# thangktran/HardwareAwareOptimalQuantumCircuitCuttingAndKnitting

Measured on AMD Instinct MI355X. Metric: subcircuit-instances/s (full-knit wall time = ms_per_step), syc 32 p=2, higher is better.
Workload: dtype f64

## Files before the change

hardwareawareoptimalquantumcircuitcuttingandknitting_amd/_lib.py:

```python
from __future__ import annotations

import ctypes
import os
import threading

_HERE = os.path.dirname(os.path.abspath(__file__))
LIB_PATH = os.environ.get("QKNIT_LIB") or os.path.join(_HERE, "libqknit.so")

c_i32, c_i64, c_u32, c_u64 = ctypes.c_int32, ctypes.c_int64, ctypes.c_uint32, ctypes.c_uint64
c_vp, c_dp, c_lp = ctypes.c_void_p, ctypes.POINTER(ctypes.c_double), ctypes.POINTER(ctypes.c_int64)


class QkPass(ctypes.Structure):
    _fields_ = [("tile_mask", c_u64), ("group_begin", c_i32), ("group_end", c_i32),
                ("flags", c_i32), ("traced_local", c_u32)]


class QkProgram(ctypes.Structure):
    _fields_ = [("n", c_i32), ("n_eff", c_i32), ("m", c_i32), ("n_slots", c_i32),
                ("packed", c_i32), ("n_passes", c_i32), ("passes", ctypes.POINTER(QkPass)),
                ("ops", c_vp), ("groups", c_vp), ("mats", c_vp)]


class QkLowrankPlan(ctypes.Structure):
# ... 42 lines not shown
    "qk_gemm_keyed": (c_i32, [c_vp, c_i64, c_i64, c_i64, c_vp, c_i64, c_vp, c_i64, c_vp, c_i64,
                              c_vp, c_i64, c_vp, ctypes.c_int]),
    "qk_gemm_keyed_pred": (c_i32, [c_vp, c_i64, c_i64, c_i64, c_vp, c_i64, c_vp, c_i64, c_vp, c_i64,
                                   c_vp, c_i64, c_vp, ctypes.c_int, c_vp]),
    "qk_gemm_outer_paired": (c_i32, [c_vp, c_i64, c_i64, c_i64, c_vp, c_i64, c_vp, c_i64, c_vp, c_i64,
                                     c_vp, c_vp]),
    "qk_knit_outer_stream": (c_i32, [c_vp, ctypes.c_int, c_i64, c_vp, c_i64, c_vp, c_i64, ctypes.c_uint64,
                                     ctypes.c_uint64, c_vp]),
    "qk_knit_outer_stream_kind": (c_i32, [ctypes.c_int, c_i64, c_u64, c_u64, c_i64, c_i64,
                                          ctypes.POINTER(ctypes.c_int), ctypes.POINTER(ctypes.c_int)]),
    "qk_knit_outer_stream_range": (c_i32, [c_vp, ctypes.c_int, c_i64, c_vp, c_i64, c_vp, c_i64, ctypes.c_uint64,
                                           ctypes.c_uint64, c_i64, c_i64, c_vp, c_vp]),
    "qk_rank_factors": (c_i32, [c_vp, c_i64, c_vp, c_vp, ctypes.c_double, ctypes.c_double, ctypes.c_double,
                                ctypes.c_int, c_vp, c_vp, c_vp]),
    "qk_prep_workspace_bytes": (c_i32, [c_vp, c_i64, c_i64, ctypes.POINTER(c_i64)]),
    "qk_prep_operands": (c_i32, [c_vp, ctypes.c_int, ctypes.c_int, c_vp, c_vp, c_i64, c_i64, c_vp, ctypes.c_int,
                                 c_vp, c_vp, c_i64, c_i64, c_vp, c_vp, c_vp, c_vp, c_vp, c_vp, c_i64]),
    "qk_compress_operands": (c_i32, [c_vp, ctypes.c_int, ctypes.c_int, c_vp, c_vp, c_i64, c_vp, c_vp, c_vp, c_i64,
                                     c_vp]),
    "qk_compress_operands_ld": (c_i32, [c_vp, ctypes.c_int, ctypes.c_int, c_vp, c_vp, c_i64, c_i64, c_vp, c_i64, c_vp,
                                        c_vp, c_i64, c_i64, c_vp, c_i64]),
    "qk_compress_probe_v": (c_i32, [c_vp, ctypes.c_int, ctypes.c_int, c_vp, c_vp, c_i64, c_i64, c_vp, c_i64, c_vp, c_vp,
                                    c_i64, c_i64, c_vp, c_i64, c_vp, c_i64, c_vp, c_i64]),
    "qk_probe_errors_vpart": (c_i32, [c_vp, ctypes.c_int, ctypes.c_int, c_vp, c_i64, c_i64, c_vp, c_i64, c_vp, c_vp,
                                      c_i64, c_vp, c_vp, ctypes.c_double, ctypes.c_double, c_vp, c_vp, c_vp, c_i64,
                                      c_vp]),
    "qk_probe_workspace_bytes": (c_i32, [c_vp, c_i64, ctypes.POINTER(c_i64)]),
    "qk_probe_errors": (c_i32, [c_vp, ctypes.c_int, ctypes.c_int, c_vp, c_i64, c_i64, c_vp, c_i64, c_vp, c_vp, c_i64,
                                c_i64, c_vp, c_i64, c_vp, c_vp, ctypes.c_double, ctypes.c_double, c_vp, c_vp, c_vp,
                                c_i64]),
    "qk_probe_errors_tally": (c_i32, [c_vp, ctypes.c_int, ctypes.c_int, c_vp, c_i64, c_i64, c_vp, c_i64, c_vp, c_vp, c_i64,
                                c_i64, c_vp, c_i64, c_vp, c_vp, ctypes.c_double, ctypes.c_double, c_vp, c_vp, c_vp,
                                c_i64, c_vp]),
    "qk_probe_accept": (c_i32, [c_vp, c_vp, ctypes.c_int, c_vp, ctypes.c_double, ctypes.c_double, c_vp, c_vp]),
    "qk_rank_tally": (c_i32, [c_vp, c_vp, c_vp, c_vp]),
    "qk_knit_workspace_bytes": (c_i32, [ctypes.POINTER(QkKnitPlan), ctypes.POINTER(c_i64)]),
    "qk_knit": (c_i32, [c_vp, ctypes.POINTER(QkKnitPlan), c_vp, c_vp, c_i64, c_vp]),
    "qk_khatri_rao": (c_i32, [c_vp, c_i64, c_i64, c_i64, c_vp, c_i64, c_vp, c_i64, c_vp]),
    "qk_gather_rows": (c_i32, [c_vp, c_i64, c_i64, c_vp, c_vp, c_vp, c_vp]),
    "qk_npd_workspace_bytes": (c_i32, [c_i64, c_i64, ctypes.POINTER(c_i64)]),
    "qk_threshold_count": (c_i32, [c_vp, c_i64, c_vp, ctypes.c_double, c_vp, c_i64, c_vp]),
    "qk_npd": (c_i32, [c_vp, c_i64, c_vp, ctypes.c_double, c_i64, c_vp, c_i64, c_vp, c_vp, c_vp]),
    "qk_qd_from_rows": (c_i32, [c_vp, c_i64, c_i64, c_vp, c_vp, ctypes.c_double, c_vp]),
    "qk_qd_merge": (c_i32, [c_vp, c_i64, c_vp, c_vp, c_i64, c_vp, c_vp, ctypes.c_double, c_i64, c_vp]),
    "qk_qd_axpby": (c_i32, [c_vp, c_i64, ctypes.c_double, c_vp, ctypes.c_double, c_vp, ctypes.c_double, c_vp]),
    "qk_hellinger": (c_i32, [c_vp, c_i64, c_vp, c_vp, c_vp]),
# ... 64 lines not shown
```

hardwareawareoptimalquantumcircuitcuttingandknitting_amd/csrc/qknit_plan.hip:

```cpp
#include <hip/hip_runtime.h>

#include <algorithm>
#include <cstdlib>
#include <string>
#include <vector>

#include "internal.h"

namespace {

int pfail(qk_ctx* ctx, int code, const std::string& msg) {
    if (ctx) ctx->err = msg;
    return code;
}

__global__ void qk_pdep_keys_kernel(int64_t n, uint64_t mask, int64_t* keys) {
    for (int64_t x = blockIdx.x * (int64_t)blockDim.x + threadIdx.x; x < n; x += (int64_t)gridDim.x * blockDim.x) {
        uint64_t m = mask, k = 0, bit = 1;
        for (; m; m &= m - 1, bit <<= 1)
            if ((uint64_t)x & bit) k |= m & (~m + 1);
        keys[x] = (int64_t)k;
    }
}

// ... 173 lines not shown
};

int lowrank_layout(qk_ctx* ctx, const qk_lowrank_plan* p, LowrankLayout& L, std::string& why) {
    if (!p || p->terms < 2 || p->terms > 64 || (p->terms & 1) || p->rows_a < 1 || p->rows_b < 1 || !p->wt_a ||
        !p->wt_b || !p->probes || p->nbits < 2 || p->nbits > 32) {
        why = "qk_knit_lowrank: need even 2 <= terms <= 64, swept rows, transforms, probes, 2 <= nbits <= 32";
        return QK_EARG;
    }
    if (p->rows_a > INT32_MAX || p->rows_b > INT32_MAX) {
        why = "qk_knit_lowrank: rows_a and rows_b must be at most INT32_MAX";
        return QK_EARG;
    }
    const uint64_t full = (uint64_t(1) << p->nbits) - 1;
    if ((p->mask_a & p->mask_b) || (p->mask_a | p->mask_b) != full || !(p->mask_b & 1)) {
        why = "qk_knit_lowrank: masks must be disjoint, cover all nbits output bits, bit 0 in mask_b";
        return QK_EARG;
    }
    const int64_t NA = int64_t(1) << __builtin_popcountll(p->mask_a), NB = int64_t(1) << __builtin_popcountll(p->mask_b);
    if (NA % 128 || NB % 128) {
        why = "qk_knit_lowrank: each fragment needs >= 7 measured clbits (operand widths multiples of 128)";
        return QK_EARG;
    }
    const int64_t K = p->terms;
    int64_t prep = 0, probe = 0;
    int rc = qk_prep_workspace_bytes(ctx, NA, NB, &prep);
    if (!rc) rc = qk_probe_workspace_bytes(ctx, NA, &probe);
    if (rc) {
        why = "qk_knit_lowrank: workspace queries failed";
        return rc;
    }
    int64_t off = 0;
    auto take = [&](int64_t bytes) { const int64_t o = off; off += align16(bytes); return o; };
    L.xa = take(K * NA * 8);
    L.xb = take(K * NB * 8);
    L.g = take(2 * K * K * 8);
    L.u = take(K * LR_PROBES * 8);
    L.prep = take(prep);
    L.ta = take(LR_RMAX * K * 8);
    L.tb = take(LR_RMAX * K * 8);
    L.r = take(8);
    L.a2 = take(LR_RMAX * NA * 8);
    L.b2 = take(LR_RMAX * NB * 8);
    L.e2 = take(2 * LR_PROBES * 8);
    L.k = take(8);
    L.err = take(8);
    L.probe = take(probe);
    L.ka = contiguous_bits(p->mask_a) ? -1 : take(NA * 8);
    L.kb = contiguous_bits(p->mask_b) ? -1 : take(NB * 8);
    L.total = off;
// ... 18 lines not shown
    return QK_OK;
}

int qk_knit_lowrank(qk_ctx* ctx, const qk_lowrank_plan* p, const double* q_a, const double* q_b, void* workspace,
                    int64_t workspace_bytes, double* out, int32_t* rank_out) {
    if (!ctx) return QK_EARG;
    LowrankLayout L;
    std::string why;
    int rc = lowrank_layout(ctx, p, L, why);
    if (rc) return pfail(ctx, rc, why);
    if (!q_a || !q_b || !out || !workspace || workspace_bytes < L.total)
        return pfail(ctx, QK_EARG, "qk_knit_lowrank: null rows / output, or workspace below qk_knit_lowrank_workspace_bytes");
    if (hipSetDevice(ctx->device) != hipSuccess) return pfail(ctx, QK_EHIP, "qk_knit_lowrank: hipSetDevice");
    char* ws = static_cast<char*>(workspace);
    auto D = [&](int64_t off) { return reinterpret_cast<double*>(ws + off); };
    const int K = p->terms;
    const int64_t NA = int64_t(1) << __builtin_popcountll(p->mask_a), NB = int64_t(1) << __builtin_popcountll(p->mask_b);
    double *XA = D(L.xa), *XB = D(L.xb), *G = D(L.g), *U = D(L.u);
    int32_t* r = reinterpret_cast<int32_t*>(ws + L.r);
    int32_t* k = reinterpret_cast<int32_t*>(ws + L.k);
    rc = qk_prep_operands(ctx, K, (int)p->rows_a, p->wt_a, q_a, NA, NA, XA, (int)p->rows_b, p->wt_b, q_b, NB, NB, XB,
                          p->probes, G, G + K * K, U, D(L.prep), L.prep_bytes);
    if (!rc) rc = qk_rank_factors(ctx, K, G, G + K * K, p->lam_tol, p->s_tol, p->s_abs, LR_RMAX, D(L.ta), D(L.tb), r);
    if (!rc) rc = qk_compress_operands(ctx, K, LR_RMAX, D(L.ta), XA, NA, D(L.a2), D(L.tb), XB, NB, D(L.b2));
    if (!rc)
        rc = qk_probe_errors(ctx, K, LR_RMAX, XA, NA, NA, D(L.a2), NA, U, D(L.b2), NB, NB, p->probes, NB, D(L.e2), r,
                             p->rank_tol, p->rank_tol_rel, k, D(L.err), D(L.probe), L.probe_bytes);
    if (!rc)
        rc = qk_knit_outer_stream_range(ctx, p->nbits, LR_RMAX, D(L.a2), NA, D(L.b2), NB, p->mask_a, p->mask_b, 0,
                                        int64_t(1) << p->nbits, k, out);
    if (rc) return rc;
    int64_t* ka = L.ka >= 0 ? reinterpret_cast<int64_t*>(ws + L.ka) : nullptr;
    int64_t* kb = L.kb >= 0 ? reinterpret_cast<int64_t*>(ws + L.kb) : nullptr;
    if (ka) hipLaunchKernelGGL(qk_pdep_keys_kernel, dim3(grid_of(NA)), dim3(256), 0, ctx->stream, NA, p->mask_a, ka);
    if (kb) hipLaunchKernelGGL(qk_pdep_keys_kernel, dim3(grid_of(NB)), dim3(256), 0, ctx->stream, NB, p->mask_b, kb);
    const int64_t sa = ka ? 0 : int64_t(1) << __builtin_ctzll(p->mask_a);
    const int64_t sb = kb ? 0 : int64_t(1) << __builtin_ctzll(p->mask_b);
    rc = qk_gemm_keyed_pred(ctx, NA, NB, K, XA, NA, XB, NB, ka, sa, kb, sb, out, 0, k);
    if (rc) return rc;
    if (rank_out) hipLaunchKernelGGL(qk_copy_i32_kernel, dim3(1), dim3(1), 0, ctx->stream, k, rank_out);
    if (hipGetLastError() != hipSuccess) return pfail(ctx, QK_EHIP, "qk_knit_lowrank: launch failed");
    return QK_OK;
}

}
```

hardwareawareoptimalquantumcircuitcuttingandknitting_amd/csrc/qknit_prep.hip:

```cpp
#include <hip/hip_runtime.h>

#include <cstdint>
#include <string>

#include "internal.h"

namespace {

typedef double d4_t __attribute__((ext_vector_type(4)));
typedef double d2_t __attribute__((ext_vector_type(2)));

constexpr int PK = 64;
constexpr int PCT = 128;
constexpr int PNP = 16;
constexpr int PTH = 512;
constexpr int XLD = PCT + 2;
constexpr int PG_BLK = 10;
constexpr int PPG = PG_BLK * 256;
constexpr int PPA = PPG;
constexpr int PPB = PPG + PK * PNP;
__host__ __device__ constexpr int prep_tri(int bi, int bj) { return bi * 4 - bi * (bi - 1) / 2 + (bj - bi); }

struct PrepSide {
    const double* Wt;
// ... 480 lines not shown
        const double* pr = P + (int64_t)i16 * ldp;
#pragma unroll
        for (int s0 = 0; s0 < 32; s0 += VB) {
            double pb[VB];
#pragma unroll
            for (int s = 0; s < VB; ++s) {
                const int64_t col = base + 4 * (s0 + s) + k4;
                pb[s] = col < N ? pr[col] : 0.0;
            }
#pragma unroll
            for (int s = 0; s < VB; ++s) {
                const double a = i16 < 8 ? Bt[wave][i16][4 * (s0 + s) + k4] : 0.0;
                va = __builtin_amdgcn_mfma_f64_16x16x4f64(a, pb[s], va, 0, 0, 0);
            }
        }
    }
#pragma unroll
    for (int r = 0; r < 2; ++r) Vw[wave][(k4 + 4 * r) * 16 + i16] = va[r];
    __syncthreads();
    if (tid < PV_PART)
        vpart[wg * PV_PART + tid] = (Vw[0][tid] + Vw[1][tid]) + (Vw[2][tid] + Vw[3][tid]);
}

__global__ __launch_bounds__(256) void qk_probe_v_kernel(int rmax, const double* __restrict__ B2, int64_t ldb2,
                                                         int64_t NB, const double* __restrict__ P, int64_t ldp,
                                                         double* __restrict__ vpart) {
    const int tid = threadIdx.x, lane = tid & 63, wave = tid >> 6;
    double acc[8][4];
#pragma unroll
    for (int jj = 0; jj < 8; ++jj)
#pragma unroll
        for (int q = 0; q < 4; ++q) acc[jj][q] = 0.0;
    struct Col {
        double b[8], pv[4];
    };
    const int64_t step = (int64_t)gridDim.x * 64;
    auto fetch = [&](int64_t c, Col& x) {
        const int64_t cc = c < NB ? c : NB - 1;
#pragma unroll
        for (int jj = 0; jj < 8; ++jj) x.b[jj] = B2[(int64_t)min(jj, rmax - 1) * ldb2 + cc];
#pragma unroll
        for (int q = 0; q < 4; ++q) x.pv[q] = P[(int64_t)(4 * wave + q) * ldp + cc];
    };
    auto mac = [&](const Col& x) {
#pragma unroll
        for (int jj = 0; jj < 8; ++jj)
// ... 91 lines not shown
            acc = __builtin_amdgcn_mfma_f64_16x16x4f64(a2[jj], Vs[4 * jj + l4][l16], acc, 0, 0, 0);
#pragma unroll
        for (int rr = 0; rr < 4; ++rr) e2 = fma(acc[rr], acc[rr], e2);
    }
    e2 += __shfl_xor(e2, 16, 64);
    e2 += __shfl_xor(e2, 32, 64);
    f2 += __shfl_xor(f2, 16, 64);
    f2 += __shfl_xor(f2, 32, 64);
    if (l4 == 0) {
        ep[wave][l16] = e2;
        ep[wave][PNP + l16] = f2;
    }
    __syncthreads();
    if (tid < 2 * PNP)
        epart[(int64_t)blockIdx.x * 2 * PNP + tid] = ep[0][tid] + ep[1][tid] + ep[2][tid] + ep[3][tid];
}

constexpr int PE = 2 * PNP;

__global__ __launch_bounds__(256) void qk_probe_accept_kernel(const double* __restrict__ epart, int n,
                                                              const int32_t* __restrict__ r_dev, double tol,
                                                              double rel_tol, double* __restrict__ e2_out,
                                                              int32_t* __restrict__ k_out, double* __restrict__ err_out,
                                                              int64_t* __restrict__ tally = nullptr) {
    __shared__ double acc[256];
    const int tid = threadIdx.x, p = tid % PE;
    constexpr int STEP = 256 / PE;
    double s8[8] = {0, 0, 0, 0, 0, 0, 0, 0};
    int b = tid / PE;
    for (; b + 31 * STEP < n; b += 32 * STEP) {
        double v[32];
#pragma unroll
        for (int u = 0; u < 32; ++u) v[u] = epart[(int64_t)(b + u * STEP) * PE + p];
#pragma unroll
        for (int u = 0; u < 32; ++u) s8[u & 7] += v[u];
    }
    for (; b < n; b += STEP) s8[0] += epart[(int64_t)b * PE + p];
    const double s = ((s8[0] + s8[1]) + (s8[2] + s8[3])) + ((s8[4] + s8[5]) + (s8[6] + s8[7]));
    acc[tid] = s;
    __syncthreads();
    for (int w = 128; w >= PE; w >>= 1) {
        if (tid < w) acc[tid] += acc[tid + w];
        __syncthreads();
    }
    if (tid < PE && e2_out) e2_out[tid] = acc[tid];
    if (tid == 0 && k_out) {
        double m = 0.0, f = 0.0;
        for (int q = 0; q < PNP; ++q) {
            m = fmax(m, acc[q]);
            f = fmax(f, acc[PNP + q]);
        }
        const double err = sqrt(m);
        const double bound = fmax(tol, rel_tol * sqrt(f));
        const int r = *r_dev;
        if (err_out) *err_out = err;
        const int k = (r > 0 && err <= bound) ? r : 0;
        *k_out = k;
        if (tally) {
            tally[0] += r == 0 ? 1 : 0;
// ... 114 lines not shown
                        double* B2, int64_t ldb2, const double* probes, int64_t ldp, double* vpart,
                        int64_t vpart_doubles) {
    if (!ctx) return QK_EARG;
    if (K < 1 || K > PK || rmax < 1 || rmax > 8 || NA < 2 || NB < 2 || (NA | NB | ldxa | lda2 | ldxb | ldb2) & 1)
        return fail(ctx, QK_EARG, "qk_compress_probe_v: need 1 <= K <= 64, 1 <= rmax <= 8, even widths and strides");
    if (ldxa < NA || lda2 < NA || ldxb < NB || ldb2 < NB || ldp < NB)
        return fail(ctx, QK_EARG, "qk_compress_probe_v: leading dimension below the width");
    if (!TA || !XA || !A2 || !TB || !XB || !B2 || !probes || !vpart)
        return fail(ctx, QK_EARG, "qk_compress_probe_v: null buffer");
    if ((reinterpret_cast<uintptr_t>(XA) | reinterpret_cast<uintptr_t>(XB) | reinterpret_cast<uintptr_t>(A2) |
         reinterpret_cast<uintptr_t>(B2)) & 15)
        return fail(ctx, QK_EARG, "qk_compress_probe_v: operands must be 16-B aligned");
    const int64_t ga = (NA + CV_COLS - 1) / CV_COLS, gb = (NB + CV_COLS - 1) / CV_COLS;
    if (vpart_doubles < gb * PV_PART) return fail(ctx, QK_EARG, "qk_compress_probe_v: vpart too small");
    if (hipSetDevice(ctx->device) != hipSuccess) return fail(ctx, QK_EHIP, "qk_compress_probe_v: hipSetDevice");
    hipLaunchKernelGGL(qk_compress_v_kernel, dim3((unsigned)(ga + gb)), dim3(256), 0, ctx->stream, K, rmax, TA, XA, NA,
                       ldxa, A2, lda2, TB, XB, NB, ldxb, B2, ldb2, probes, ldp, vpart, (int)ga);
    const hipError_t e = hipGetLastError();
    if (e != hipSuccess)
        return fail(ctx, QK_EHIP, (std::string("qk_compress_probe_v: ") + hipGetErrorString(e)).c_str());
    return QK_OK;
}

int qk_probe_errors_vpart(qk_ctx* ctx, int K, int rmax, const double* XA, int64_t ldx, int64_t NA, const double* A2,
                          int64_t lda2, const double* U, const double* vpart, int64_t gv, double* e2,
                          const int32_t* r_dev, double tol, double rel_tol, int32_t* k_out, double* err_out,
                          double* work, int64_t work_bytes, int64_t* tally) {
    if (!ctx) return QK_EARG;
    if (K < 1 || K > PK || rmax < 1 || rmax > 8 || NA < 16 || NA % 16 || gv < 1)
        return fail(ctx, QK_EARG, "qk_probe_errors_vpart: need 1 <= K <= 64, 1 <= rmax <= 8, NA % 16 == 0, gv >= 1");
    if (!XA || !A2 || !U || !vpart || !work || (k_out && !r_dev) || (tally && !k_out))
        return fail(ctx, QK_EARG, "qk_probe_errors_vpart: null buffer");
    if (ldx < NA) return fail(ctx, QK_EARG, "qk_probe_errors_vpart: leading dimension");
    const int gd = probe_grid_d(ctx, NA);
    if (work_bytes < (int64_t)(PV_GRID * PV_PART + gd * PE) * (int64_t)sizeof(double))
        return fail(ctx, QK_EARG, "qk_probe_errors_vpart: workspace too small (qk_probe_workspace_bytes)");
    if (hipSetDevice(ctx->device) != hipSuccess) return fail(ctx, QK_EHIP, "qk_probe_errors_vpart: hipSetDevice");
    double* epart = work + PV_GRID * PV_PART;
    hipLaunchKernelGGL(qk_probe_d_kernel, dim3(gd), dim3(256), 0, ctx->stream, K, rmax, XA, ldx, NA, A2, lda2, U, vpart,
                       (int)gv, epart);
    hipLaunchKernelGGL(qk_probe_accept_kernel, dim3(1), dim3(256), 0, ctx->stream, epart, gd, r_dev, tol, rel_tol, e2,
                       k_out, err_out, tally);
    const hipError_t e = hipGetLastError();
    if (e != hipSuccess)
        return fail(ctx, QK_EHIP, (std::string("qk_probe_errors_vpart: ") + hipGetErrorString(e)).c_str());
    return QK_OK;
// ... 79 lines not shown
```

hardwareawareoptimalquantumcircuitcuttingandknitting_amd/engine.py:

```python
from __future__ import annotations

import atexit
import contextlib
import ctypes
import dataclasses
import hashlib
import logging
import os
import threading
from dataclasses import dataclass, field
from time import perf_counter

import numpy as np

from . import _lib
from .fragment_program import (FragmentProgram, JobTable, basis_reduce, build_jobs, compile_fragment,
                               dedup_labels)
from .knit_plan import LabelSpace, deposit_keys, factor_vgate
from .sweep_plan import K_SLOT, EncodedProgram, encode

_torch = None


def torch():
# ... 1282 lines not shown
    A2 = ab[:rmax * NA].view(rmax, NA)
    B2 = ab[rmax * NA:].view(rmax, NB)
    base, n = (0, NA) if a_cols is None else a_cols
    assert 0 <= base and n >= 1 and base + n <= NA and XA.shape[1] in (n, NA)
    src = XA.data_ptr() if XA.shape[1] == n else XA.data_ptr() + 8 * base
    if a_cols is not None and POISON_UNUSED:
        A2.fill_(float("nan"))
    gv = -(-NB // CV_COLS)
    vpart = T.empty((gv, 8, N_PROBES), dtype=T.float64, device=XA.device)
    ctx.check(ctx.lib.qk_compress_probe_v(ctx.handle, K, rmax, TA.data_ptr(), src, n, XA.stride(0),
                                          A2.data_ptr() + 8 * base, NA, TB.data_ptr(), XB.data_ptr(), NB, NB,
                                          B2.data_ptr(), NB, probes.data_ptr(), NB, vpart.data_ptr(), vpart.numel()),
              "qk_compress_probe_v")
    return A2, B2, vpart


def compress_probe_v_ok(XA, XB, a_cols=None) -> bool:
    n = XA.shape[1] if a_cols is None else a_cols[1]
    base = 0 if a_cols is None or XA.shape[1] == n else a_cols[0]
    return (n % 2 == 0 and XB.shape[1] % 2 == 0 and XA.stride(0) % 2 == 0 and base % 2 == 0
            and (XA.data_ptr() + 8 * base) % 16 == 0 and XB.data_ptr() % 16 == 0)


_PROBE_WORK: dict = {}
def probe_errors(ctx: Context, XA, A2, U, B2, probes, r=None, tol: float = 0.0, a2_cols: tuple | None = None,
                 rel_tol: float = 0.0, tally=None, vpart=None):
    T = torch()
    K, NA = XA.shape
    rmax = A2.shape[0]
    NB = B2.shape[1]
    assert U.shape == (K, N_PROBES) and probes.shape == (N_PROBES, NB) and B2.shape[0] == rmax
    assert all(t.is_contiguous() for t in (A2, U, B2, probes))
    assert XA.stride(1) == 1 and XA.stride(0) >= NA
    off = 0 if a2_cols is None else a2_cols[0]
    assert (a2_cols is None and A2.shape[1] == NA) or (a2_cols is not None and a2_cols[1] == NA)
    dev = XA.device
    need = ctypes.c_int64()
    ctx.check(ctx.lib.qk_probe_workspace_bytes(ctx.handle, NA, ctypes.byref(need)), "qk_probe_workspace_bytes")
    key = (str(dev), T.cuda.current_stream(dev).cuda_stream)
    work = _PROBE_WORK.get(key)
    if work is None or work.numel() * 8 < need.value:
        work = _PROBE_WORK[key] = T.empty(max(need.value // 8, 1), dtype=T.float64, device=dev)
    e2 = T.empty(2 * N_PROBES, dtype=T.float64, device=dev)
    k = T.empty(1, dtype=T.int32, device=dev) if r is not None else None
    err = T.empty(1, dtype=T.float64, device=dev) if r is not None else None
    assert tally is None or (r is not None and tally.dtype == T.int64 and tally.numel() == 4)
# ... 411 lines not shown
```

hardwareawareoptimalquantumcircuitcuttingandknitting_amd/pipeline.py:

```python
from __future__ import annotations

import ctypes
import os
import threading
from dataclasses import dataclass
from time import perf_counter

import numpy as np

from . import _lib, engine
from .fragment_program import JobTable


_PROBES: dict = {}
_PROBES_LOCK = threading.Lock()


def _mm_nt(X, Y):
    L = X.shape[1]
    nb = L // 256 if L % 256 == 0 else 1
    if nb <= 1:
        return X @ Y.T
    Xb = X.view(X.shape[0], nb, 256).transpose(0, 1)
    Yb = Y.reshape(Y.shape[0], nb, 256).transpose(0, 1)
# ... 114 lines not shown
        for k, i in enumerate(low):
            t |= ((o >> (len(high) + k)) & 1) << i
        perm[o] = t
    return perm


def _joined(T, a, b):
    base = a._base
    if (base is not None and b._base is base and base.dim() == 1 and a.is_contiguous() and b.is_contiguous()
            and a.data_ptr() == base.data_ptr()
            and b.data_ptr() == a.data_ptr() + a.numel() * a.element_size()
            and base.numel() == a.numel() + b.numel()):
        return base
    return T.cat([a.reshape(-1), b.reshape(-1)])


class Backend:

    REQUIRED = ("prepare_fragments", "upload_jobs", "workspace_bytes", "empty", "zeros", "to_device", "sweep",
                "reduce_labels", "gather_rows", "gemm_keyed", "khatri_rao", "event")
    ROUTES = {
        "rank_factors": ("rank_factors", "compress", "probe_errors"),
        "prep_operands": ("prep_operands",),
        "sweep_rows": ("sweep_rows",),
        "plan_multi": ("plan_multi", "sweep_multi"),
        "knit_select": ("knit_select", "npd_pairs"),
        "out_buffer": ("out_buffer",),
        "knit_outer_stream": ("knit_outer_stream",),
        "gemm_outer_paired": ("gemm_outer_paired",),
    }
    OPTIONAL = ("sweep_labels", "fold_traced", "probe_accept", "select_above", "npd_dense")
    routes: frozenset = frozenset()
    dev = None
    fuses_tally = False
    shared_init = None

    def __init_subclass__(cls, **kw):
        super().__init_subclass__(**kw)
        needs = cls.REQUIRED + tuple(op for r in cls.routes for op in cls.ROUTES[r])
        known = (set(cls.REQUIRED) | set(cls.OPTIONAL) | {op for ops in cls.ROUTES.values() for op in ops}
                 | {n for n, v in vars(Backend).items() if callable(v)})
        bad = ([f"missing {n}" for n in needs if not callable(getattr(cls, n, None))]
               + [f"{n} is not a Backend operation" for n, v in vars(cls).items()
                  if callable(v) and not n.startswith("_") and n not in known])
        if bad:
            raise TypeError(f"{cls.__name__}: " + "; ".join(bad))
# ... 131 lines not shown
        return engine.khatri_rao(self.ctx, A, B)

    def gemm_outer_paired(self, A, B, keyB, **kw):
        return engine.gemm_outer_paired(self.ctx, A, B, keyB, **kw)

    def knit_outer_stream(self, A, B, clbits_a, clbits_b, nbits, out, o_begin=0, o_count=None, k_dev=None):
        return engine.knit_outer_stream(self.ctx, A, B, clbits_a, clbits_b, nbits, out, o_begin=o_begin,
                                        o_count=o_count, k_dev=k_dev)

    def outer_stream_kernel(self, K, clbits_a, clbits_b, nbits, o_begin=0, o_count=None):
        return engine.knit_outer_stream_kernel(K, clbits_a, clbits_b, nbits, o_begin, o_count)

    def rank_factors(self, GA, GB):
        return engine.rank_factors_device(self.ctx, GA, GB)

    def prep_operands(self, WtA, qA, WtB, qB, probes):
        return engine.prep_operands(self.ctx, WtA, qA, WtB, qB, probes)

    fuses_tally = True

    def probe_errors(self, XA, A2, U, B2, probes, r=None, tol=0.0, a2_cols=None, rel_tol=0.0, tally=None, vpart=None):
        return engine.probe_errors(self.ctx, XA, A2, U, B2, probes, r=r, tol=tol, a2_cols=a2_cols, rel_tol=rel_tol,
                                   tally=tally, vpart=vpart)

    def compress_v(self, TA, XA, TB, XB, probes, a_cols=None, a_width=None):
        if os.environ.get("QKNIT_COMPRESS_V", "1") == "0" or not engine.compress_probe_v_ok(XA, XB, a_cols):
            return None
        return engine.compress_probe_v(self.ctx, TA, XA, TB, XB, probes, a_cols=a_cols, a_width=a_width)

    def probe_accept(self, e2, r, tol, rel_tol=0.0):
        return engine.probe_accept(self.ctx, e2, r, tol, rel_tol)

    def rank_tally(self, r, k, acc):
        self.ctx.check(self.ctx.lib.qk_rank_tally(self.ctx.handle, r.data_ptr(), k.data_ptr(), acc.data_ptr()),
                       "qk_rank_tally")

    def compress(self, TA, XA, TB, XB, a_cols=None, a_width=None):
        return engine.compress_operands(self.ctx, TA, XA, TB, XB, a_cols=a_cols, a_width=a_width)

    def knit_select(self, A, B, clbits_a, clbits_b, nbits, accuracy, k_dev=None):
        return engine.knit_select(self.ctx, A, B, clbits_a, clbits_b, nbits, accuracy, k_dev=k_dev)

    def npd_pairs(self, keys, vals):
        return engine.npd_pairs(self.ctx, keys, vals)

    def select_above(self, dense, accuracy, key_base=0):
# ... 571 lines not shown
            self._note_rank(r, k_eff)
        return k_eff, err

    def _prep_dev_rank(self, qs) -> PreparedStep:
        ia, ib = self.order[0], self.order[-1]
        if self._fused_prep(qs):
            x = self._probes(qs[ib].shape[1], qs[ib].device)
            mats, G, U = self._prep_fused(qs, x)
            TA, TB, r = self.be.rank_factors(G[0], G[1])
            return self._compress_and_check(TA, TB, r, mats, U, x)
        mats = self.operands(qs)
        self.last_prep = "torch"
        A, B = mats[ia], mats[ib]
        G = self.T.stack([_mm_nt(A, A), _mm_nt(B, B)])
        TA, TB, r = self.be.rank_factors(G[0].contiguous(), G[1].contiguous())
        A2, B2 = (TA @ A).contiguous(), (TB @ B).contiguous()
        k_eff, _ = self._accept(A, B, A2, B2, self._probes(B.shape[1], B.device), r)
        return PreparedStep(A2, B2, k_eff, mats)

    def _compress_and_check(self, TA, TB, r, mats, U, x) -> PreparedStep:
        ia, ib = self.order[0], self.order[-1]
        a_cols = self._replicated_a_cols()
        kw = {"a_cols": a_cols} if a_cols is not None else {}
        cv = self.be.compress_v(TA, mats[ia], TB, mats[ib], x, **kw)
        check = {}
        if cv is not None:
            A2, B2, check["vpart"] = cv
        else:
            A2, B2 = self.be.compress(TA, mats[ia], TB, mats[ib], **kw)
        XA = mats[ia]
        if a_cols is not None:
            XA = XA[:, a_cols[0]:a_cols[0] + a_cols[1]]
            check["a2_cols"] = a_cols
        tally = self.be.fuses_tally
        if tally:
            check["tally"] = self._tally_for(r.device)
        _, k_eff, _ = self.be.probe_errors(XA, A2, U, B2, x, r=r, tol=self.rank_tol, rel_tol=self.rank_tol_rel,
                                           **check)
        if tally:
            self._pending += 1
        else:
            self._note_rank(r, k_eff)
        return PreparedStep(A2, B2, k_eff, mats)

    def _launch_dev_rank(self, p: PreparedStep):
        ia, ib = self.order[0], self.order[-1]
# ... 690 lines not shown
```

include/qknit.h:

```cpp
#ifndef QKNIT_H
#define QKNIT_H

#include <stdint.h>

#ifdef __cplusplus
extern "C" {
#endif

#define QK_OK 0
#define QK_EARG 1
#define QK_EHIP 2
#define QK_ESTATE 3

#define QK_TILE_BITS 12
#define QK_FIBER_BITS 4

enum { QK_U1 = 0, QK_D1 = 1, QK_SLOT = 2, QK_U2 = 3, QK_D2 = 4, QK_CX = 5, QK_SWAP = 6, QK_SCALE = 7,
       QK_U1R = 8, QK_U1X = 9, QK_D1R = 10, QK_D2R = 11, QK_SCALER = 12 };

typedef struct qk_op {
    int32_t kind;
    int32_t a, b;
    int32_t e1, e2;
    int32_t slot;
// ... 150 lines not shown
int qk_allreduce(qk_ctx* ctx, qk_comm* comm, const double* send, double* recv, int64_t count);
int qk_reduce(qk_ctx* ctx, qk_comm* comm, const double* send, double* recv, int64_t count, int root);
int qk_allgather(qk_ctx* ctx, qk_comm* comm, const double* send, double* recv, int64_t count);
int qk_alltoall(qk_ctx* ctx, qk_comm* comm, const double* send, double* recv, int64_t count);

int qk_rank_factors(qk_ctx* ctx, int64_t K, const double* GA, const double* GB, double lam_tol, double s_tol,
                    double s_abs, int rmax, double* TA, double* TB, int32_t* r_out);

int qk_prep_workspace_bytes(qk_ctx* ctx, int64_t NA, int64_t NB, int64_t* bytes);
int qk_prep_operands(qk_ctx* ctx, int K, int RA, const double* WtA, const double* qA, int64_t ldqA, int64_t NA,
                     double* XA, int RB, const double* WtB, const double* qB, int64_t ldqB, int64_t NB, double* XB,
                     const double* probes, double* GA, double* GB, double* U, double* work, int64_t work_bytes);

int qk_compress_operands(qk_ctx* ctx, int K, int rmax, const double* TA, const double* XA, int64_t NA, double* A2,
                         const double* TB, const double* XB, int64_t NB, double* B2);
int qk_compress_operands_ld(qk_ctx* ctx, int K, int rmax, const double* TA, const double* XA, int64_t NA, int64_t ldxa,
                            double* A2, int64_t lda2, const double* TB, const double* XB, int64_t NB, int64_t ldxb,
                            double* B2, int64_t ldb2);

int qk_compress_probe_v(qk_ctx* ctx, int K, int rmax, const double* TA, const double* XA, int64_t NA, int64_t ldxa,
                        double* A2, int64_t lda2, const double* TB, const double* XB, int64_t NB, int64_t ldxb,
                        double* B2, int64_t ldb2, const double* probes, int64_t ldp, double* vpart,
                        int64_t vpart_doubles);

int qk_probe_errors_vpart(qk_ctx* ctx, int K, int rmax, const double* XA, int64_t ldx, int64_t NA, const double* A2,
                          int64_t lda2, const double* U, const double* vpart, int64_t gv, double* e2,
                          const int32_t* r_dev, double tol, double rel_tol, int32_t* k_out, double* err_out,
                          double* work, int64_t work_bytes, int64_t* tally);

int qk_probe_workspace_bytes(qk_ctx* ctx, int64_t NA, int64_t* bytes);
int qk_probe_errors(qk_ctx* ctx, int K, int rmax, const double* XA, int64_t ldx, int64_t NA, const double* A2,
                    int64_t lda2, const double* U, const double* B2, int64_t ldb2, int64_t NB, const double* probes,
                    int64_t ldp, double* e2, const int32_t* r_dev, double tol, double rel_tol, int32_t* k_out,
                    double* err_out, double* work, int64_t work_bytes);
int qk_probe_errors_tally(qk_ctx* ctx, int K, int rmax, const double* XA, int64_t ldx, int64_t NA, const double* A2,
                          int64_t lda2, const double* U, const double* B2, int64_t ldb2, int64_t NB,
                          const double* probes, int64_t ldp, double* e2, const int32_t* r_dev, double tol,
                          double rel_tol, int32_t* k_out, double* err_out, double* work, int64_t work_bytes,
                          int64_t* tally);
int qk_probe_accept(qk_ctx* ctx, const double* e2, int n, const int32_t* r_dev, double tol, double rel_tol,
                    int32_t* k_out, double* err_out);
int qk_rank_tally(qk_ctx* ctx, const int32_t* r_dev, const int32_t* k_dev, int64_t* acc);


int qk_npd_workspace_bytes(int64_t n, int64_t count, int64_t* bytes);

// ... 67 lines not shown
```

Measured before the change: 519,400.

## Fuse operand compression with low-rank probe error check in one kernel

```diff
diff --git a/hardwareawareoptimalquantumcircuitcuttingandknitting_amd/_lib.py b/hardwareawareoptimalquantumcircuitcuttingandknitting_amd/_lib.py
--- a/hardwareawareoptimalquantumcircuitcuttingandknitting_amd/_lib.py
+++ b/hardwareawareoptimalquantumcircuitcuttingandknitting_amd/_lib.py
@@ -88,6 +88,10 @@
                                         c_vp, c_i64, c_i64, c_vp, c_i64]),
     "qk_compress_probe_v": (c_i32, [c_vp, ctypes.c_int, ctypes.c_int, c_vp, c_vp, c_i64, c_i64, c_vp, c_i64, c_vp, c_vp,
                                     c_i64, c_i64, c_vp, c_i64, c_vp, c_i64, c_vp, c_i64]),
+    "qk_compress_check_workspace_bytes": (c_i32, [c_vp, c_i64, ctypes.POINTER(c_i64)]),
+    "qk_compress_check": (c_i32, [c_vp, ctypes.c_int, ctypes.c_int, c_vp, c_vp, c_i64, c_i64, c_vp, c_i64, c_vp, c_vp,
+                                  c_i64, c_i64, c_vp, c_i64, c_vp, c_vp, ctypes.c_double, ctypes.c_double, c_vp, c_vp,
+                                  c_vp, c_vp, c_vp, c_i64]),
     "qk_probe_errors_vpart": (c_i32, [c_vp, ctypes.c_int, ctypes.c_int, c_vp, c_i64, c_i64, c_vp, c_i64, c_vp, c_vp,
                                       c_i64, c_vp, c_vp, ctypes.c_double, ctypes.c_double, c_vp, c_vp, c_vp, c_i64,
                                       c_vp]),
diff --git a/hardwareawareoptimalquantumcircuitcuttingandknitting_amd/csrc/qknit_plan.hip b/hardwareawareoptimalquantumcircuitcuttingandknitting_amd/csrc/qknit_plan.hip
--- a/hardwareawareoptimalquantumcircuitcuttingandknitting_amd/csrc/qknit_plan.hip
+++ b/hardwareawareoptimalquantumcircuitcuttingandknitting_amd/csrc/qknit_plan.hip
@@ -219,9 +219,11 @@
         return QK_EARG;
     }
     const int64_t K = p->terms;
-    int64_t prep = 0, probe = 0;
+    int64_t prep = 0, probe = 0, check = 0;
     int rc = qk_prep_workspace_bytes(ctx, NA, NB, &prep);
     if (!rc) rc = qk_probe_workspace_bytes(ctx, NA, &probe);
+    if (!rc) rc = qk_compress_check_workspace_bytes(ctx, NA, &check);
+    probe = probe > check ? probe : check;
     if (rc) {
         why = "qk_knit_lowrank: workspace queries failed";
         return rc;
@@ -286,8 +288,13 @@
     rc = qk_prep_operands(ctx, K, (int)p->rows_a, p->wt_a, q_a, NA, NA, XA, (int)p->rows_b, p->wt_b, q_b, NB, NB, XB,
                           p->probes, G, G + K * K, U, D(L.prep), L.prep_bytes);
     if (!rc) rc = qk_rank_factors(ctx, K, G, G + K * K, p->lam_tol, p->s_tol, p->s_abs, LR_RMAX, D(L.ta), D(L.tb), r);
-    if (!rc) rc = qk_compress_operands(ctx, K, LR_RMAX, D(L.ta), XA, NA, D(L.a2), D(L.tb), XB, NB, D(L.b2));
-    if (!rc)
+    const char* cc_env = getenv("QKNIT_COMPRESS_CHECK");
+    const bool fused = !(cc_env && cc_env[0] == '0' && !cc_env[1]) && !(reinterpret_cast<uintptr_t>(ws) & 15);
+    if (!rc && fused)
+        rc = qk_compress_check(ctx, K, LR_RMAX, D(L.ta), XA, NA, NA, D(L.a2), NA, D(L.tb), XB, NB, NB, D(L.b2), NB, U, r,
+                               p->rank_tol, p->rank_tol_rel, D(L.e2), k, D(L.err), nullptr, D(L.probe), L.probe_bytes);
+    if (!rc && !fused) rc = qk_compress_operands(ctx, K, LR_RMAX, D(L.ta), XA, NA, D(L.a2), D(L.tb), XB, NB, D(L.b2));
+    if (!rc && !fused)
         rc = qk_probe_errors(ctx, K, LR_RMAX, XA, NA, NA, D(L.a2), NA, U, D(L.b2), NB, NB, p->probes, NB, D(L.e2), r,
                              p->rank_tol, p->rank_tol_rel, k, D(L.err), D(L.probe), L.probe_bytes);
     if (!rc)
diff --git a/hardwareawareoptimalquantumcircuitcuttingandknitting_amd/csrc/qknit_prep.hip b/hardwareawareoptimalquantumcircuitcuttingandknitting_amd/csrc/qknit_prep.hip
--- a/hardwareawareoptimalquantumcircuitcuttingandknitting_amd/csrc/qknit_prep.hip
+++ b/hardwareawareoptimalquantumcircuitcuttingandknitting_amd/csrc/qknit_prep.hip
@@ -526,6 +526,195 @@
         vpart[wg * PV_PART + tid] = (Vw[0][tid] + Vw[1][tid]) + (Vw[2][tid] + Vw[3][tid]);
 }
 
+constexpr int CC_SR = 8;
+constexpr int CC_LD = 128 + 16;
+struct CheckLds {
+    __attribute__((aligned(16))) double Tt[PK][8];
+    __attribute__((aligned(16))) double St[4][CC_SR][CC_LD];
+    double Us[PK][PNP];
+    double Tb[8][PK];
+    double Vh[PV_PART];
+    double Vs[8][PNP];
+    double ep[4][2 * PNP];
+};
+
+template <bool CHECK>
+__device__ __forceinline__ void compress_check_side(CheckLds& L, int K, int rmax, const double* __restrict__ Tg,
+                                                    const double* __restrict__ X, int64_t N, int64_t ld,
+                                                    double* __restrict__ out, int64_t ldo,
+                                                    const double* __restrict__ TB, const double* __restrict__ U,
+                                                    const int32_t* __restrict__ r_dev, double* __restrict__ epart,
+                                                    int64_t wg) {
+    const int tid = threadIdx.x, lane = tid & 63, wave = tid >> 6;
+    const int64_t base = wg * CV_COLS + wave * 128;
+    const int64_t c = base + 2 * lane;
+    const bool valid = c < N;
+    const int64_t cl = valid ? c : N - 2;
+    d2_t acc[8];
+#pragma unroll
+    for (int j = 0; j < 8; ++j) acc[j] = (d2_t){0.0, 0.0};
+    d2_t buf[2][PCW];
+    auto load = [&](int ch, d2_t (&b)[PCW]) {
+#pragma unroll
+        for (int u = 0; u < PCW; ++u) {
+            const int k = min(ch * PCW + u, K - 1);
+            b[u] = *reinterpret_cast<const d2_t*>(X + (int64_t)k * ld + cl);
+        }
+    };
+    const int nch = (K + PCW - 1) / PCW;
+    {
+        double tv[2], tb[2] = {0.0, 0.0}, uv[4] = {0.0, 0.0, 0.0, 0.0};
+        int rv = rmax;
+#pragma unroll
+        for (int i = 0; i < 2; ++i) {
+            const int e = tid + 256 * i, k = e >> 3, j = e & 7;
+            tv[i] = Tg[min(j, rmax - 1) * K + min(k, K - 1)];
+        }
+        if (CHECK) {
+#pragma unroll
+            for (int i = 0; i < 2; ++i) {
+                const int e = tid + 256 * i, j = e >> 6, k = e & 63;
+                tb[i] = TB[min(j, rmax - 1) * K + min(k, K - 1)];
+            }
+#pragma unroll
+            for (int i = 0; i < 4; ++i) uv[i] = U[min(tid + 256 * i, K * PNP - 1)];
+            if (r_dev) rv = *r_dev;
+        }
+        if (base < N) load(0, buf[0]);
+#pragma unroll
+        for (int i = 0; i < 2; ++i) {
+            const int e = tid + 256 * i, k = e >> 3, j = e & 7;
+            L.Tt[k][j] = (k < K && j < rmax) ? tv[i] : 0.0;
+        }
+        if (CHECK) {
+            const int rows = rv < rmax ? rv : rmax;
+#pragma unroll
+            for (int i = 0; i < 2; ++i) {
+                const int e = tid + 256 * i, j = e >> 6, k = e & 63;
+                L.Tb[j][k] = (k < K && j < rows) ? tb[i] : 0.0;
+            }
+#pragma unroll
+            for (int i = 0; i < 4; ++i) {
+                const int e = tid + 256 * i;
+                L.Us[e / PNP][e % PNP] = e < K * PNP ? uv[i] : 0.0;
+            }
+        }
+    }
+    auto lds_barrier = [] {
+        asm volatile("s_waitcnt lgkmcnt(0)" ::: "memory");
+        __builtin_amdgcn_s_barrier();
+    };
+    lds_barrier();
+    if (CHECK) {
+        const int e = tid & (PV_PART - 1), h = tid >> 7, j = e / PNP, p = e % PNP;
+        double s = 0.0;
+#pragma unroll
+        for (int k = 0; k < PK / 2; ++k) s = fma(L.Tb[j][32 * h + k], L.Us[32 * h + k][p], s);
+        if (h == 1) L.Vh[e] = s;
+        lds_barrier();
+        if (h == 0) L.Vs[j][p] = -(s + L.Vh[e]);
+        lds_barrier();
+    }
+    const int l16 = lane & 15, l4 = lane >> 4;
+    double e2 = 0.0, f2 = 0.0;
+    if (base < N) {
+        d4_t dacc[8];
+#pragma unroll
+        for (int b = 0; b < 8; ++b) dacc[b] = (d4_t){0.0, 0.0, 0.0, 0.0};
+#pragma unroll
+        for (int ch = 0; ch < PK / PCW; ++ch) {
+            if (ch >= nch) break;
+            if (ch + 1 < nch) load(ch + 1, buf[(ch + 1) & 1]);
+#pragma unroll
+            for (int u = 0; u < PCW; ++u) {
+                const int k = ch * PCW + u;
+                double t[8];
+#pragma unroll
+                for (int h = 0; h < 4; ++h) {
+                    const d2_t tv = *reinterpret_cast<const d2_t*>(&L.Tt[k][2 * h]);
+                    t[2 * h] = tv.x;
+                    t[2 * h + 1] = tv.y;
+                }
+#pragma unroll
+                for (int j = 0; j < 8; ++j) {
+                    acc[j].x = fma(t[j], buf[ch & 1][u].x, acc[j].x);
+                    acc[j].y = fma(t[j], buf[ch & 1][u].y, acc[j].y);
+                }
+            }
+            if (CHECK) {
+#pragma unroll
+                for (int hf = 0; hf < PCW / CC_SR; ++hf) {
+#pragma unroll
+                    for (int u = 0; u < CC_SR; ++u)
+                        *reinterpret_cast<d2_t*>(&L.St[wave][u][2 * lane]) =
+                            valid ? buf[ch & 1][hf * CC_SR + u] : (d2_t){0.0, 0.0};
+                    __builtin_amdgcn_wave_barrier();
+#pragma unroll
+                    for (int kk = 0; kk < CC_SR / 4; ++kk) {
+                        const double ub = L.Us[ch * PCW + hf * CC_SR + 4 * kk + l4][l16];
+#pragma unroll
+                        for (int b = 0; b < 8; ++b)
+                            dacc[b] = __builtin_amdgcn_mfma_f64_16x16x4f64(L.St[wave][4 * kk + l4][16 * b + l16], ub,
+                                                                           dacc[b], 0, 0, 0);
+                    }
+                    __builtin_amdgcn_wave_barrier();
+                }
+            }
+        }
+        if (valid) {
+#pragma unroll
+            for (int j = 0; j < 8; ++j)
+                if (j < rmax) *reinterpret_cast<d2_t*>(out + (int64_t)j * ldo + c) = acc[j];
+        }
+        if (CHECK) {
+#pragma unroll
+            for (int j = 0; j < 8; ++j)
+                *reinterpret_cast<d2_t*>(&L.St[wave][j][2 * lane]) = (valid && j < rmax) ? acc[j] : (d2_t){0.0, 0.0};
+            __builtin_amdgcn_wave_barrier();
+#pragma unroll
+            for (int b = 0; b < 8; ++b) {
+                d4_t d = dacc[b];
+#pragma unroll
+                for (int rr = 0; rr < 4; ++rr) f2 = fma(d[rr], d[rr], f2);
+#pragma unroll
+                for (int jj = 0; jj < 2; ++jj)
+                    d = __builtin_amdgcn_mfma_f64_16x16x4f64(L.St[wave][4 * jj + l4][16 * b + l16],
+                                                             L.Vs[4 * jj + l4][l16], d, 0, 0, 0);
+#pragma unroll
+                for (int rr = 0; rr < 4; ++rr) e2 = fma(d[rr], d[rr], e2);
+            }
+        }
+    }
+    if (!CHECK) return;
+    e2 += __shfl_xor(e2, 16, 64);
+    e2 += __shfl_xor(e2, 32, 64);
+    f2 += __shfl_xor(f2, 16, 64);
+    f2 += __shfl_xor(f2, 32, 64);
+    if (l4 == 0) {
+        L.ep[wave][l16] = e2;
+        L.ep[wave][PNP + l16] = f2;
+    }
+    __syncthreads();
+    if (tid < 2 * PNP) epart[wg * 2 * PNP + tid] = L.ep[0][tid] + L.ep[1][tid] + L.ep[2][tid] + L.ep[3][tid];
+}
+
+__global__ __launch_bounds__(256) void qk_compress_check_kernel(int K, int rmax, const double* __restrict__ TA,
+                                                                const double* __restrict__ XA, int64_t NA, int64_t ldxa,
+                                                                double* __restrict__ A2, int64_t lda2,
+                                                                const double* __restrict__ TB,
+                                                                const double* __restrict__ XB, int64_t NB, int64_t ldxb,
+                                                                double* __restrict__ B2, int64_t ldb2,
+                                                                const double* __restrict__ U,
+                                                                const int32_t* __restrict__ r_dev,
+                                                                double* __restrict__ epart, int nA_wg) {
+    __shared__ CheckLds L;
+    if ((int)blockIdx.x >= nA_wg)
+        compress_check_side<false>(L, K, rmax, TB, XB, NB, ldxb, B2, ldb2, nullptr, nullptr, nullptr, nullptr,
+                                   (int64_t)blockIdx.x - nA_wg);
+    else
+        compress_check_side<true>(L, K, rmax, TA, XA, NA, ldxa, A2, lda2, TB, U, r_dev, epart, (int64_t)blockIdx.x);
+}
+
 __global__ __launch_bounds__(256) void qk_probe_v_kernel(int rmax, const double* __restrict__ B2, int64_t ldb2,
                                                          int64_t NB, const double* __restrict__ P, int64_t ldp,
                                                          double* __restrict__ vpart) {
@@ -663,7 +852,7 @@
                                                               const int32_t* __restrict__ r_dev, double tol,
                                                               double rel_tol, double* __restrict__ e2_out,
                                                               int32_t* __restrict__ k_out, double* __restrict__ err_out,
-                                                              int64_t* __restrict__ tally = nullptr) {
+                                                              int64_t* __restrict__ tally = nullptr, int mid = 0) {
     __shared__ double acc[256];
     const int tid = threadIdx.x, p = tid % PE;
     constexpr int STEP = 256 / PE;
@@ -676,6 +865,14 @@
 #pragma unroll
         for (int u = 0; u < 32; ++u) s8[u & 7] += v[u];
     }
+    if (mid)
+        for (; b + 7 * STEP < n; b += 8 * STEP) {
+            double v[8];
+#pragma unroll
+            for (int u = 0; u < 8; ++u) v[u] = epart[(int64_t)(b + u * STEP) * PE + p];
+#pragma unroll
+            for (int u = 0; u < 8; ++u) s8[u] += v[u];
+        }
     for (; b < n; b += STEP) s8[0] += epart[(int64_t)b * PE + p];
     const double s = ((s8[0] + s8[1]) + (s8[2] + s8[3])) + ((s8[4] + s8[5]) + (s8[6] + s8[7]));
     acc[tid] = s;
@@ -836,6 +1033,41 @@
     return QK_OK;
 }
 
+int qk_compress_check_workspace_bytes(qk_ctx* ctx, int64_t NA, int64_t* bytes) {
+    if (!ctx || !bytes) return QK_EARG;
+    if (NA < 1) return fail(ctx, QK_EARG, "qk_compress_check_workspace_bytes: need NA >= 1");
+    *bytes = ((NA + CV_COLS - 1) / CV_COLS) * PE * (int64_t)sizeof(double);
+    return QK_OK;
+}
+
+int qk_compress_check(qk_ctx* ctx, int K, int rmax, const double* TA, const double* XA, int64_t NA, int64_t ldxa,
+                      double* A2, int64_t lda2, const double* TB, const double* XB, int64_t NB, int64_t ldxb,
+                      double* B2, int64_t ldb2, const double* U, const int32_t* r_dev, double tol, double rel_tol,
+                      double* e2, int32_t* k_out, double* err_out, int64_t* tally, double* work, int64_t work_bytes) {
+    if (!ctx) return QK_EARG;
+    if (K < 1 || K > PK || rmax < 1 || rmax > 8 || NA < 2 || NB < 2 || (NA | NB | ldxa | lda2 | ldxb | ldb2) & 1)
+        return fail(ctx, QK_EARG, "qk_compress_check: need 1 <= K <= 64, 1 <= rmax <= 8, even widths and strides");
+    if (ldxa < NA || lda2 < NA || ldxb < NB || ldb2 < NB)
+        return fail(ctx, QK_EARG, "qk_compress_check: leading dimension below the width");
+    if (!TA || !XA || !A2 || !TB || !XB || !B2 || !U || !work || (k_out && !r_dev) || (tally && !k_out))
+        return fail(ctx, QK_EARG, "qk_compress_check: null buffer");
+    if ((reinterpret_cast<uintptr_t>(XA) | reinterpret_cast<uintptr_t>(XB) | reinterpret_cast<uintptr_t>(A2) |
+         reinterpret_cast<uintptr_t>(B2)) & 15)
+        return fail(ctx, QK_EARG, "qk_compress_check: operands must be 16-B aligned");
+    const int64_t ga = (NA + CV_COLS - 1) / CV_COLS, gb = (NB + CV_COLS - 1) / CV_COLS;
+    if (ga + gb > INT32_MAX) return fail(ctx, QK_EARG, "qk_compress_check: too many columns for one launch");
+    if (work_bytes < ga * PE * (int64_t)sizeof(double))
+        return fail(ctx, QK_EARG, "qk_compress_check: workspace too small (qk_compress_check_workspace_bytes)");
+    if (hipSetDevice(ctx->device) != hipSuccess) return fail(ctx, QK_EHIP, "qk_compress_check: hipSetDevice");
+    hipLaunchKernelGGL(qk_compress_check_kernel, dim3((unsigned)(ga + gb)), dim3(256), 0, ctx->stream, K, rmax, TA, XA,
+                       NA, ldxa, A2, lda2, TB, XB, NB, ldxb, B2, ldb2, U, r_dev, work, (int)ga);
+    hipLaunchKernelGGL(qk_probe_accept_kernel, dim3(1), dim3(256), 0, ctx->stream, work, (int)ga, r_dev, tol, rel_tol,
+                       e2, k_out, err_out, tally, 1);
+    const hipError_t e = hipGetLastError();
+    if (e != hipSuccess) return fail(ctx, QK_EHIP, (std::string("qk_compress_check: ") + hipGetErrorString(e)).c_str());
+    return QK_OK;
+}
+
 int qk_probe_errors_vpart(qk_ctx* ctx, int K, int rmax, const double* XA, int64_t ldx, int64_t NA, const double* A2,
                           int64_t lda2, const double* U, const double* vpart, int64_t gv, double* e2,
                           const int32_t* r_dev, double tol, double rel_tol, int32_t* k_out, double* err_out,
diff --git a/hardwareawareoptimalquantumcircuitcuttingandknitting_amd/engine.py b/hardwareawareoptimalquantumcircuitcuttingandknitting_amd/engine.py
--- a/hardwareawareoptimalquantumcircuitcuttingandknitting_amd/engine.py
+++ b/hardwareawareoptimalquantumcircuitcuttingandknitting_amd/engine.py
@@ -1328,6 +1328,45 @@
             and (XA.data_ptr() + 8 * base) % 16 == 0 and XB.data_ptr() % 16 == 0)
 
 
+_CHECK_WORK: dict = {}
+
+
+def compress_check(ctx: Context, TA, XA, TB, XB, U, r=None, tol: float = 0.0, rel_tol: float = 0.0, tally=None,
+                   a_cols: tuple | None = None, a_width: int | None = None):
+    T = torch()
+    rmax, K = TA.shape
+    assert TB.shape == (rmax, K) and XA.shape[0] == K and XB.shape[0] == K and U.shape == (K, N_PROBES)
+    assert XA.stride(1) == 1 and all(t.is_contiguous() for t in (XB, TA, TB, U))
+    NA = XA.shape[1] if a_width is None else a_width
+    NB = XB.shape[1]
+    dev = XA.device
+    ab = T.empty(rmax * (NA + NB), dtype=T.float64, device=dev)
+    A2 = ab[:rmax * NA].view(rmax, NA)
+    B2 = ab[rmax * NA:].view(rmax, NB)
+    base, n = (0, NA) if a_cols is None else a_cols
+    assert 0 <= base and n >= 1 and base + n <= NA and XA.shape[1] in (n, NA)
+    src = XA.data_ptr() if XA.shape[1] == n else XA.data_ptr() + 8 * base
+    if a_cols is not None and POISON_UNUSED:
+        A2.fill_(float("nan"))
+    need = ctypes.c_int64()
+    ctx.check(ctx.lib.qk_compress_check_workspace_bytes(ctx.handle, n, ctypes.byref(need)),
+              "qk_compress_check_workspace_bytes")
+    key = (str(dev), T.cuda.current_stream(dev).cuda_stream)
+    work = _CHECK_WORK.get(key)
+    if work is None or work.numel() * 8 < need.value:
+        work = _CHECK_WORK[key] = T.empty(max(need.value // 8, 1), dtype=T.float64, device=dev)
+    e2 = T.empty(2 * N_PROBES, dtype=T.float64, device=dev)
+    k = T.empty(1, dtype=T.int32, device=dev) if r is not None else None
+    err = T.empty(1, dtype=T.float64, device=dev) if r is not None else None
+    assert tally is None or (r is not None and tally.dtype == T.int64 and tally.numel() == 4)
+    ctx.check(ctx.lib.qk_compress_check(ctx.handle, K, rmax, TA.data_ptr(), src, n, XA.stride(0),
+                                        A2.data_ptr() + 8 * base, NA, TB.data_ptr(), XB.data_ptr(), NB, NB,
+                                        B2.data_ptr(), NB, U.data_ptr(), _ptr(r), tol, rel_tol, e2.data_ptr(), _ptr(k),
+                                        _ptr(err), _ptr(tally), work.data_ptr(), work.numel() * 8),
+              "qk_compress_check")
+    return A2, B2, e2, k, err
+
+
 _PROBE_WORK: dict = {}
 def probe_errors(ctx: Context, XA, A2, U, B2, probes, r=None, tol: float = 0.0, a2_cols: tuple | None = None,
                  rel_tol: float = 0.0, tally=None, vpart=None):
diff --git a/hardwareawareoptimalquantumcircuitcuttingandknitting_amd/pipeline.py b/hardwareawareoptimalquantumcircuitcuttingandknitting_amd/pipeline.py
--- a/hardwareawareoptimalquantumcircuitcuttingandknitting_amd/pipeline.py
+++ b/hardwareawareoptimalquantumcircuitcuttingandknitting_amd/pipeline.py
@@ -160,6 +160,7 @@
     ROUTES = {
         "rank_factors": ("rank_factors", "compress", "probe_errors"),
         "prep_operands": ("prep_operands",),
+        "compress_check": ("compress_check",),
         "sweep_rows": ("sweep_rows",),
         "plan_multi": ("plan_multi", "sweep_multi"),
         "knit_select": ("knit_select", "npd_pairs"),
@@ -337,6 +338,13 @@
     def probe_errors(self, XA, A2, U, B2, probes, r=None, tol=0.0, a2_cols=None, rel_tol=0.0, tally=None, vpart=None):
         return engine.probe_errors(self.ctx, XA, A2, U, B2, probes, r=r, tol=tol, a2_cols=a2_cols, rel_tol=rel_tol,
                                    tally=tally, vpart=vpart)
+
+    def compress_check(self, TA, XA, TB, XB, U, r, tol=0.0, rel_tol=0.0, tally=None, a_cols=None):
+        if os.environ.get("QKNIT_COMPRESS_CHECK", "1") == "0" or not engine.compress_probe_v_ok(XA, XB, a_cols):
+            return None
+        A2, B2, _, k, err = engine.compress_check(self.ctx, TA, XA, TB, XB, U, r=r, tol=tol, rel_tol=rel_tol,
+                                                  tally=tally, a_cols=a_cols)
+        return A2, B2, k, err
 
     def compress_v(self, TA, XA, TB, XB, probes, a_cols=None, a_width=None):
         if os.environ.get("QKNIT_COMPRESS_V", "1") == "0" or not engine.compress_probe_v_ok(XA, XB, a_cols):
@@ -954,6 +962,17 @@
         ia, ib = self.order[0], self.order[-1]
         a_cols = self._replicated_a_cols()
         kw = {"a_cols": a_cols} if a_cols is not None else {}
+        if "compress_check" in self.be.routes:
+            tally = self._tally_for(r.device) if self.be.fuses_tally else None
+            cc = self.be.compress_check(TA, mats[ia], TB, mats[ib], U, r, tol=self.rank_tol, rel_tol=self.rank_tol_rel,
+                                        tally=tally, **kw)
+            if cc is not None:
+                A2, B2, k_eff, _ = cc
+                if tally is not None:
+                    self._pending += 1
+                else:
+                    self._note_rank(r, k_eff)
+                return PreparedStep(A2, B2, k_eff, mats)
         cv = self.be.compress_v(TA, mats[ia], TB, mats[ib], x, **kw)
         check = {}
         if cv is not None:
diff --git a/include/qknit.h b/include/qknit.h
--- a/include/qknit.h
+++ b/include/qknit.h
@@ -196,6 +196,12 @@
                         double* A2, int64_t lda2, const double* TB, const double* XB, int64_t NB, int64_t ldxb,
                         double* B2, int64_t ldb2, const double* probes, int64_t ldp, double* vpart,
                         int64_t vpart_doubles);
+
+int qk_compress_check_workspace_bytes(qk_ctx* ctx, int64_t NA, int64_t* bytes);
+int qk_compress_check(qk_ctx* ctx, int K, int rmax, const double* TA, const double* XA, int64_t NA, int64_t ldxa,
+                      double* A2, int64_t lda2, const double* TB, const double* XB, int64_t NB, int64_t ldxb,
+                      double* B2, int64_t ldb2, const double* U, const int32_t* r_dev, double tol, double rel_tol,
+                      double* e2, int32_t* k_out, double* err_out, int64_t* tally, double* work, int64_t work_bytes);
 
 int qk_probe_errors_vpart(qk_ctx* ctx, int K, int rmax, const double* XA, int64_t ldx, int64_t NA, const double* A2,
                           int64_t lda2, const double* U, const double* vpart, int64_t gv, double* e2,
```

After: 520,700, median of 6. No clear change (+0.3%).
